# gssales/gaussian-splatting-reflection

Measured on AMD Instinct MI355X. Metric: train_step_views_per_s (fwd+bwd, 1e6 Gaussians @1080p, surfel rasterizer + reflection path), higher is better.
Workload: dtype f32

## Files before the change

gaussian-splatting-reflection_amd/csrc/gsr_common.hip:

```cpp
#include "gsr_internal.hpp"
#include <cstdarg>
#include <string>
#include <initializer_list>
#include <vector>
#include <mutex>
#include "gsr_sort.hpp"
#include <rocprim/device/device_scan.hpp>
#include <rocprim/iterator/counting_iterator.hpp>
#include <rocprim/iterator/transform_iterator.hpp>

namespace gsr {

static thread_local char g_err[512] = "";
void set_error(const char* fmt, ...) {
	va_list ap;
	va_start(ap, fmt);
	vsnprintf(g_err, sizeof(g_err), fmt, ap);
	va_end(ap);
}


struct ProfRec {
	int stage;
	hipEvent_t e0, e1;
};
static bool g_prof_on = false;
static std::vector<ProfRec*> g_prof_recs;
static std::vector<ProfRec*> g_prof_free;
static std::mutex g_prof_mu;

StageTimer::StageTimer(int stage_, hipStream_t stream_) : stage(stage_), stream(stream_), rec(nullptr) {
	if (!g_prof_on) return;
	std::lock_guard<std::mutex> lk(g_prof_mu);
	ProfRec* r = nullptr;
	if (!g_prof_free.empty()) {
		r = g_prof_free.back();
		g_prof_free.pop_back();
	} else {
		r = new ProfRec();
		if (hipEventCreate(&r->e0) != hipSuccess || hipEventCreate(&r->e1) != hipSuccess) { delete r; return; }
	}
	r->stage = stage;
	(void)hipEventRecord(r->e0, stream);
	rec = r;
}
StageTimer::~StageTimer() {
	if (!rec) return;
	ProfRec* r = (ProfRec*)rec;
	(void)hipEventRecord(r->e1, stream);
	std::lock_guard<std::mutex> lk(g_prof_mu);
	g_prof_recs.push_back(r);
}

static int g_opt_cull = 1;
int option_cull() { return g_opt_cull; }
static int g_opt_dev = 0;
int option_dev() { return g_opt_dev; }
static int g_opt_emit_items = 0;
static int g_opt_mailbox = 1;
static int option_mailbox() { return g_opt_mailbox; }
static int g_opt_sort_driver = GSR_ONESWEEP_DRIVER;
int option_sort_driver() { return GSR_ONESWEEP_DRIVER && g_opt_sort_driver; }

uint32_t higher_msb(uint32_t n) {
	uint32_t msb = sizeof(n) * 4;
	uint32_t step = msb;
	while (step > 1) {
		step /= 2;
		if (n >> msb) msb += step;
		else msb -= step;
	}
	if (n >> msb) msb++;
	return msb;
}

using SortConfig = rocprim::radix_sort_config<rocprim::default_config, rocprim::default_config, rocprim::default_config, 65536>;
#ifndef DEPTH_SORT_BS
#define DEPTH_SORT_BS 1024
#endif
#ifndef DEPTH_SORT_IPT
#define DEPTH_SORT_IPT 4
#endif
#define DEPTH_SORT_SHAPE DEPTH_SORT_BS, DEPTH_SORT_IPT, 8
#define DEPTH_KEY_BITS 31u
#define DEPTH_KEY_PLACES 4u
#ifndef TILE_SORT_IPT
#define TILE_SORT_IPT 16
#endif
#ifndef TILE_SORT_BITS
#define TILE_SORT_BITS 8
#endif
#ifndef TILE_SORT_BS
#define TILE_SORT_BS 1024
#endif
#define TILE_SORT_SHAPE TILE_SORT_BS, TILE_SORT_IPT, TILE_SORT_BITS
#ifndef TILE_SORT_SMALL_FROM
#define TILE_SORT_SMALL_FROM 9000000
#endif
#define TILE_SORT_SHAPE_SMALL TILE_SORT_BS, (TILE_SORT_IPT / 2), TILE_SORT_BITS
#define TILE_SORT_SHAPE_SMALL7 TILE_SORT_BS, (TILE_SORT_IPT / 2), 7
static bool tile_sort_small(size_t R) { return R >= (size_t)TILE_SORT_SMALL_FROM; }
static bool tile_sort_7bit(size_t R, int end_bit) { return tile_sort_small(R) && end_bit > 7 && end_bit <= 14; }
template <class F>
static auto with_tile_sort(size_t R, int end_bit, F&& f) {
	if (tile_sort_7bit(R, end_bit)) return f(RadixSort<TILE_SORT_SHAPE_SMALL7, SortConfig>{});
	if (tile_sort_small(R)) return f(RadixSort<TILE_SORT_SHAPE_SMALL, SortConfig>{});
	return f(RadixSort<TILE_SORT_SHAPE, SortConfig>{});
}
using DepthSort = RadixSort<DEPTH_SORT_SHAPE, SortConfig>;

struct OrderRect {
	const uint32_t* rect;
	int packed;
	__host__ __device__ unsigned long long operator()(uint32_t i) const {
		uint32_t hi = 0u;
// ... 465 lines not shown
int run_tile_order(const ImageState& img, size_t tiles, hipStream_t stream) {
	if (tiles == 0) return 0;
	tile_order_kernel<<<1, 1024, 0, stream>>>((int)tiles, img.ranges, img.tile_order);
	GSR_LAUNCH_CHECK(0, stream);
	return 0;
}

__global__ void __launch_bounds__(256) mark_visible_kernel(int P, const float* __restrict__ pts, const float* __restrict__ vm,
                                                           uint8_t* __restrict__ present) {
#pragma clang fp contract(off)
	const int idx = blockIdx.x * 256 + threadIdx.x;
	if (idx >= P) return;
	const float x = pts[3 * idx], y = pts[3 * idx + 1], z = pts[3 * idx + 2];
	const float pz = vm[2] * x + vm[6] * y + vm[10] * z + vm[14];
	present[idx] = (pz <= 0.2f) ? 0 : 1;
}

__global__ void __launch_bounds__(256) widen_clamped_kernel(int P, const uint8_t* __restrict__ packed, uint8_t* __restrict__ out) {
	const int idx = blockIdx.x * 256 + threadIdx.x;
	if (idx >= P) return;
	const uint8_t b = packed[idx];
	out[3 * idx + 0] = b & 1;
	out[3 * idx + 1] = (b >> 1) & 1;
	out[3 * idx + 2] = (b >> 2) & 1;
}
struct RecPick { int n; int pos[9]; };
__global__ void __launch_bounds__(256) pick_rec_kernel(int P, const float* __restrict__ rec, int stride, RecPick pick, float* __restrict__ out) {
	const int i = blockIdx.x * 256 + threadIdx.x;
	if (i >= P * pick.n) return;
	const int idx = i / pick.n, k = i % pick.n;
	out[i] = rec[(size_t)idx * stride + pick.pos[k]];
}
__global__ void __launch_bounds__(256) gather_rec_kernel(int P, const float* __restrict__ rec, int stride, int first, int nf,
                                                         float* __restrict__ out) {
	const int i = blockIdx.x * 256 + threadIdx.x;
	if (i >= P * nf) return;
	const int idx = i / nf, k = i % nf;
	out[i] = rec[(size_t)idx * stride + first + k];
}

}

using namespace gsr;

extern "C" const char* gsr_last_error(void) { return g_err; }
extern "C" int gsr_version(void) { return GSR_ABI_VERSION; }


extern "C" int gsr_set_option(const char* name, int value) {
	if (std::string(name) == "cull") { g_opt_cull = value ? 1 : 0; return 0; }
	if (std::string(name) == "dev") { g_opt_dev = value; return 0; }
	if (std::string(name) == "emit_items") { g_opt_emit_items = (value == 1 || value == 2) ? value : 0; return 0; }
	if (std::string(name) == "mailbox") { g_opt_mailbox = value ? 1 : 0; return 0; }
	if (std::string(name) == "sort_driver") { g_opt_sort_driver = value ? 1 : 0; return 0; }
	set_error("gsr_set_option: unknown option '%s'", name);
	return GSR_E_INVALID;
}
extern "C" int gsr_profile_enable(int on) {
	std::lock_guard<std::mutex> lk(g_prof_mu);
	for (ProfRec* r : g_prof_recs) g_prof_free.push_back(r);
	g_prof_recs.clear();
	g_prof_on = on != 0;
	return 0;
}
extern "C" int gsr_profile_collect(float* ms_out, int* launches_out) {
	std::lock_guard<std::mutex> lk(g_prof_mu);
	for (int i = 0; i < GSR_STAGE_COUNT; i++) { if (ms_out) ms_out[i] = 0.f; if (launches_out) launches_out[i] = 0; }
	for (ProfRec* r : g_prof_recs) {
		float ms = 0.f;
		if (hipEventSynchronize(r->e1) == hipSuccess && hipEventElapsedTime(&ms, r->e0, r->e1) == hipSuccess) {
			if (ms_out) ms_out[r->stage] += ms;
			if (launches_out) launches_out[r->stage] += 1;
		}
		g_prof_free.push_back(r);
	}
	g_prof_recs.clear();
	return 0;
}

extern "C" int gsr_mark_visible(int P, const float* means3D, const float* viewmatrix, const float* projmatrix, uint8_t* present,
                                void* stream_) {
	(void)projmatrix;
	hipStream_t stream = (hipStream_t)stream_;
	if (P < 0 || (P > 0 && (!means3D || !viewmatrix || !present))) { set_error("gsr_mark_visible: invalid argument"); return GSR_E_INVALID; }
	if (P == 0) return 0;
	mark_visible_kernel<<<(P + 255) / 256, 256, 0, stream>>>(P, means3D, viewmatrix, present);
	GSR_LAUNCH_CHECK(0, stream);
	return 0;
}

extern "C" int gsr_debug_fetch(int variant, const char* name, int P, int R, int width, int height, const void* geom_buffer,
                               const void* binning_buffer, const void* image_buffer, void* dst, void* stream_) {
	hipStream_t stream = (hipStream_t)stream_;
	const int tiles_x = (width + 15) / 16, tiles_y = (height + 15) / 16;
	const size_t HW = (size_t)width * height, tiles = (size_t)tiles_x * tiles_y;
	const WorkspaceLayout& layout = variant == 0 ? SURFEL_LAYOUT : GAUSS_LAYOUT;
	const int stride = layout.rec_f4 * 4;
	GeomState g = carve_geom((void*)geom_buffer, P, layout, nullptr);
	ImageState im = carve_image((void*)image_buffer, HW, tiles, layout, nullptr);
	BinningState b = carve_binning((void*)binning_buffer, R, tiles, 0, nullptr);
	auto d2d = [&](const void* src, size_t bytes) -> int {
		if (bytes == 0) return 0;
		GSR_HIP_CHECK(hipMemcpyAsync(dst, src, bytes, hipMemcpyDeviceToDevice, stream));
		return 0;
	};
	auto gather = [&](int first, int nf) -> int {
// ... 53 lines not shown
```

gaussian-splatting-reflection_amd/csrc/gsr_internal.hpp:

```cpp
#pragma once
#include <cstring>
#include <cstdint>
#include <cstdio>
#include <hip/hip_runtime.h>
#include "../../include/gsr_hip.h"

#define GSR_TILE 16
#define GSR_TILE_PIX 256

namespace gsr {

void set_error(const char* fmt, ...);
#define GSR_HIP_CHECK(expr)                                                                       \
	do {                                                                                          \
		hipError_t _e = (expr);                                                                   \
		if (_e != hipSuccess) {                                                                   \
			gsr::set_error("%s failed: %s (%s:%d)", #expr, hipGetErrorString(_e), __FILE__, __LINE__); \
			return GSR_E_HIP;                                                                     \
		}                                                                                         \
	} while (0)
#define GSR_LAUNCH_CHECK(debug, stream)                                  \
	do {                                                                 \
		GSR_HIP_CHECK(hipGetLastError());                                \
		if (debug) GSR_HIP_CHECK(hipStreamSynchronize(stream));          \
// ... 79 lines not shown
constexpr WorkspaceLayout SURFEL_LAYOUT{S_REC_F4, 0, S_ACC_F, 3, 2};
constexpr WorkspaceLayout GAUSS_LAYOUT{G_REC_F4, 0, G_ACC_F, 1, 1};

GeomState carve_geom(void* buf, size_t P, const WorkspaceLayout& layout, size_t* total);
ImageState carve_image(void* buf, size_t HW, size_t tiles, const WorkspaceLayout& layout, size_t* total);
BinningState carve_binning(void* buf, size_t R, size_t tiles, size_t sort_temp_bytes, size_t* total, bool blend_masks = true);
int forward_workspace(gsr_alloc_fn alloc, void* alloc_user, const WorkspaceLayout& layout, size_t P, size_t HW, size_t tiles, GeomState* geom,
                      ImageState* img);

static inline int check_sh_input(const char* entry, int D, int M, const float* shs) {
	if (D < 0 || D > 3 || (shs && (D + 1) * (D + 1) > M)) { set_error("%s: SH degree %d not supported with M=%d", entry, D, M); return GSR_E_INVALID; }
	if (shs && ((M * 3) & 3) == 0 && misaligned16(shs)) {
		set_error("%s: shs (rows of a multiple of 16 bytes) must be 16-byte aligned (float4 accesses); got %p", entry, (const void*)shs);
		return GSR_E_INVALID;
	}
	return 0;
}

struct RasterCam {
	const float* view;
	const float* proj;
	const float* campos;
	int W, H;
	float tan_fovx, tan_fovy, focal_x, focal_y;
};
static inline RasterCam make_cam(const float* view, const float* proj, const float* campos, int W, int H, float tan_fovx, float tan_fovy) {
	RasterCam c;
	c.view = view; c.proj = proj; c.campos = campos; c.W = W; c.H = H;
	c.tan_fovx = tan_fovx; c.tan_fovy = tan_fovy;
	c.focal_y = H / (2.0f * tan_fovy);
	c.focal_x = W / (2.0f * tan_fovx);
	return c;
}

struct BackwardWorkspace { GeomState geom; ImageState img; BinningState bin; int tiles_x, ntiles; };
static inline int backward_prologue(const char* entry, const char* func, const WorkspaceLayout& layout, int P, int M, int R, int width, int height,
                                    bool missing_pointer, const float* shs, const float* dL_dsh, const float* dL_drot, const float* also_aligned,
                                    const char* also_what, void* geom_buffer, void* binning_buffer, void* image_buffer, hipStream_t stream,
                                    BackwardWorkspace* w) {
	if (P < 0 || R < 0 || width <= 0 || height <= 0) { set_error("%s: invalid size", entry); return GSR_E_INVALID; }
	if (P == 0) return 0;
	if (missing_pointer) { set_error("%s: missing required pointer", entry); return GSR_E_INVALID; }
	if (shs && ((M * 3) & 3) == 0) GSR_REQUIRE_ALIGNED16_IN(func, shs, "shs (rows of a multiple of 16 bytes)");
	if (shs && ((M * 3) & 3) == 0) GSR_REQUIRE_ALIGNED16_IN(func, dL_dsh, "dL_dsh");
	GSR_REQUIRE_ALIGNED16_IN(func, dL_drot, "dL_drot");
	GSR_REQUIRE_ALIGNED16_IN(func, also_aligned, also_what);
	w->tiles_x = (width + 15) / 16;
	w->ntiles = w->tiles_x * ((height + 15) / 16);
	w->geom = carve_geom(geom_buffer, P, layout, nullptr);
	w->img = carve_image(image_buffer, (size_t)width * height, w->ntiles, layout, nullptr);
	w->bin = carve_binning(binning_buffer, R, w->ntiles, 0, nullptr);
	GSR_HIP_CHECK(hipMemsetAsync(w->geom.acc, 0, (size_t)P * layout.acc_floats * sizeof(float), stream));
	return 1;
}

int option_cull();
int option_dev();
size_t sort_temp_bytes(size_t R, int end_bit);
int run_tile_order(const ImageState& img, size_t tiles, hipStream_t stream);
uint32_t higher_msb(uint32_t n);

int run_binning(gsr_alloc_fn alloc, void* alloc_user, int P, int tiles_x, int tiles_y, const GeomState& geom,
                const ImageState& img, BinningState* out_binning, int prefiltered, int debug, hipStream_t stream, bool blend_masks = true);

int side_gate_wait(hipStream_t stream);
int refl_sort_keys_early(uint32_t L, int width, int height, float* scratch, size_t scratch_floats, const uint32_t* sort_keys, int async, bool gated,
                         hipStream_t stream);

}

#ifdef __HIPCC__
namespace gsr {

__device__ __forceinline__ int f2i(float v) { return (int)v; }

__device__ __forceinline__ void get_rect(float px, float py, int max_radius, int gx, int gy, uint32_t& x0, uint32_t& y0,
                                         uint32_t& x1, uint32_t& y1) {
	const float r = (float)max_radius;
	x0 = (uint32_t)min(gx, max(0, f2i((px - r) / 16.0f)));
	y0 = (uint32_t)min(gy, max(0, f2i((py - r) / 16.0f)));
	x1 = (uint32_t)min(gx, max(0, f2i((px + r + 15.0f) / 16.0f)));
	y1 = (uint32_t)min(gy, max(0, f2i((py + r + 15.0f) / 16.0f)));
}

#define GSR_DPP1(CTRL, i) "v_add_f32_dpp %" #i ", %" #i ", %" #i " " CTRL "\n\t"
#define GSR_DPP4(CTRL) GSR_DPP1(CTRL, 0) GSR_DPP1(CTRL, 1) GSR_DPP1(CTRL, 2) GSR_DPP1(CTRL, 3)
#define GSR_SHR1 "row_shr:1 row_mask:0xf bank_mask:0xf bound_ctrl:0"
#define GSR_SHR2 "row_shr:2 row_mask:0xf bank_mask:0xf bound_ctrl:0"
#define GSR_SHR4 "row_shr:4 row_mask:0xf bank_mask:0xf bound_ctrl:0"
#define GSR_SHR8 "row_shr:8 row_mask:0xf bank_mask:0xf bound_ctrl:0"
#define GSR_BC15 "row_bcast:15 row_mask:0xa bank_mask:0xf"
#define GSR_BC31 "row_bcast:31 row_mask:0xc bank_mask:0xf"
__device__ __forceinline__ void wave_sum4(float* v) {
	asm volatile("s_nop 1\n\t" GSR_DPP4(GSR_SHR1) GSR_DPP4(GSR_SHR2) GSR_DPP4(GSR_SHR4) GSR_DPP4(GSR_SHR8) GSR_DPP4(GSR_BC15) GSR_DPP4(GSR_BC31)
	             : "+v"(v[0]), "+v"(v[1]), "+v"(v[2]), "+v"(v[3]));
}

#define GSR_Q1(CTRL, i) "v_add_f32_dpp %" #i ", %" #i ", %" #i " " CTRL " row_mask:0xf bank_mask:0xf\n\t"
#define GSR_DPPB(CTRL, BANK, dst, src) "v_add_f32_dpp %" #dst ", %" #src ", %" #src " " CTRL " row_mask:0xf bank_mask:" BANK "\n\t"
#define GSR_L1(CTRL, d, a, b) GSR_DPPB(CTRL, "0x3", d, a) GSR_DPPB(CTRL, "0xc", d, b)
__device__ __forceinline__ void row_reduce20(const float* v, float* z) {
	float p0, q0, p1, q1, p2, q2, p3, q3, p4, q4;
	asm volatile("s_nop 1\n\t" GSR_L1("row_mirror", 0, 6, 7) GSR_L1("row_mirror", 1, 8, 9) GSR_L1("row_mirror", 2, 10, 11)
	             GSR_L1("row_mirror", 3, 12, 13) GSR_L1("row_mirror", 4, 14, 15) GSR_L1("row_mirror", 5, 16, 17)
	             : "=&v"(p0), "=&v"(q0), "=&v"(p1), "=&v"(q1), "=&v"(p2), "=&v"(q2)
	             : "v"(v[0]), "v"(v[1]), "v"(v[2]), "v"(v[3]), "v"(v[4]), "v"(v[5]), "v"(v[6]), "v"(v[7]), "v"(v[8]), "v"(v[9]), "v"(v[10]), "v"(v[11]));
// ... 202 lines not shown
```

gaussian-splatting-reflection_amd/csrc/gsr_surfel.hip:

```cpp
#include <type_traits>
#include "gsr_internal.hpp"
#include "gsr_tile_walk.hpp"
#include "gsr_sort.hpp"
#include "gsr_math.hpp"
#include "gsr_refl.hpp"

namespace gsr {

#define SA_COLOR 0
#define SA_REFL 3
#define SA_NORMAL 4
#define SA_OPAC 7
#define SA_T 8
#define SA_MEAN2D 17

#define S_NEAR 0.2f
#define S_FAR 100.0f
#define S_FILTER_INV_SQ 2.0f

__device__ __forceinline__ M3 quat_to_rotmat(const float* __restrict__ q, float& w, float& x, float& y, float& z) {
#pragma clang fp contract(off)
	const float s = 1.0f / sqrtf(q[3] * q[3] + q[0] * q[0] + q[1] * q[1] + q[2] * q[2]);
	w = q[0] * s; x = q[1] * s; y = q[2] * s; z = q[3] * s;
	return m3_make(1.f - 2.f * (y * y + z * z), 2.f * (x * y + w * z), 2.f * (x * z - w * y), 2.f * (x * y - w * z),
// ... 24 lines not shown
	float qw, qx, qy, qz;
	const M3 R = quat_to_rotmat(rot, qw, qx, qy, qz);
	const float s0 = mod * scale[0], s1 = mod * scale[1];
	const float L0[3] = {R.m[0][0] * s0, R.m[0][1] * s0, R.m[0][2] * s0};
	const float L1[3] = {R.m[1][0] * s1, R.m[1][1] * s1, R.m[1][2] * s1};
	const float* pm = cam.proj;
	float AB[4][3];
#pragma unroll
	for (int j = 0; j < 4; j++) {
		AB[j][0] = L0[0] * pm[j] + L0[1] * pm[j + 4] + L0[2] * pm[j + 8];
		AB[j][1] = L1[0] * pm[j] + L1[1] * pm[j + 4] + L1[2] * pm[j + 8];
		AB[j][2] = px * pm[j] + py * pm[j + 4] + pz * pm[j + 8] + pm[j + 12];
	}
	const float Wh = (float)(float(cam.W) / 2.0), Wm = (float)(float(cam.W - 1) / 2.0);
	const float Hh = (float)(float(cam.H) / 2.0), Hm = (float)(float(cam.H - 1) / 2.0);
#pragma unroll
	for (int i = 0; i < 3; i++) {
		T.m[0][i] = AB[0][i] * Wh + AB[3][i] * Wm;
		T.m[1][i] = AB[1][i] * Hh + AB[3][i] * Hm;
		T.m[2][i] = AB[3][i];
	}
	const float* vm = cam.view;
	const float nx = R.m[2][0], ny = R.m[2][1], nz = R.m[2][2];
	normal = f3(vm[0] * nx + vm[4] * ny + vm[8] * nz, vm[1] * nx + vm[5] * ny + vm[9] * nz, vm[2] * nx + vm[6] * ny + vm[10] * nz);
}

__device__ __forceinline__ void surfel_cull_record(const M3& T, float cx, float cy, float opa, float4& c0, float4& c1) {
	c0 = make_float4(cx, cy, 0.f, 0.f);
	c1 = make_float4(0.f, cx, cy, -2.0f);
	if (!(opa >= 1.0f / 255.0f)) return;
	const float c2f = 2.0f * logf(255.0f * opa) * 1.05f + 0.1f;
	c1.w = 0.5f * c2f * 1.02f;
	const double ic2 = 1.0 / (double)c2f;
	const double a00 = T.m[0][0], a01 = T.m[0][1], a02 = T.m[0][2];
	const double a10 = T.m[1][0], a11 = T.m[1][1], a12 = T.m[1][2];
	const double a20 = T.m[2][0], a21 = T.m[2][1], a22 = T.m[2][2];
	const double sigma = a20 * a20 + a21 * a21 - a22 * a22 * ic2;
	if (!(sigma < -1e-6 * a22 * a22 * ic2)) return;
	const double sx = a00 * a20 + a01 * a21 - a02 * a22 * ic2, sy = a10 * a20 + a11 * a21 - a12 * a22 * ic2;
	const double Sxx = a00 * a00 + a01 * a01 - a02 * a02 * ic2, Sxy = a00 * a10 + a01 * a11 - a02 * a12 * ic2,
	             Syy = a10 * a10 + a11 * a11 - a12 * a12 * ic2;
	const double is = 1.0 / sigma;
	const double ex = sx * is, ey = sy * is;
	const double g = -is * 1.0404;
	const double Vxx = (Sxx - sx * sx * is) * g + 0.25, Vxy = (Sxy - sx * sy * is) * g, Vyy = (Syy - sy * sy * is) * g + 0.25;
	const double det = Vxx * Vyy - Vxy * Vxy;
	if (!(Vxx > 0.25) || !(Vyy > 0.25) || !(det > 0.0)) return;
	const float fa = (float)(Vyy / det), fb = (float)(-Vxy / det), fc = (float)(Vxx / det);
	if (!(fa > 0.f) || !(fc > 0.f) || !(fa * fc - fb * fb > 0.f) || !(fabsf((float)ex) < 1e7f) || !(fabsf((float)ey) < 1e7f)) return;
	c0 = make_float4((float)ex, (float)ey, fa, fb);
	c1.x = fc;
}

template <bool TRAIN>
__device__ __forceinline__ bool
surfel_preprocess_one(int idx, int D, int M, const float* __restrict__ means, const float* __restrict__ scales, float scale_modifier,
                      const float* __restrict__ rotations, const float* __restrict__ opacities, const float* __restrict__ shs,
                      const float* __restrict__ transMat_precomp, const float* __restrict__ colors_precomp, const float* __restrict__ refl,
                      const uint8_t* __restrict__ env_scope_mask, const RasterCam& cam, int* __restrict__ radii, const GeomState& g, int gx, int gy,
                      int prefiltered, float* __restrict__ gaussian_weights, float4* o) {
#pragma clang fp contract(off)
	radii[idx] = 0;
	if constexpr (TRAIN) gaussian_weights[idx] = 0.f;
	g.tiles_touched[idx] = 0;
	reinterpret_cast<uint2*>(g.rect)[idx] = make_uint2(0u, 0u);
	g.depths[idx] = __int_as_float(0x7f7fffff);
	const float mx = means[3 * idx], my = means[3 * idx + 1], mz = means[3 * idx + 2];
	const float* vm = cam.view;
	const float pvx = vm[0] * mx + vm[4] * my + vm[8] * mz + vm[12];
	const float pvy = vm[1] * mx + vm[5] * my + vm[9] * mz + vm[13];
	const float pvz = vm[2] * mx + vm[6] * my + vm[10] * mz + vm[14];
	if (pvz <= 0.2f) {
		if (prefiltered) g.flags[0] = 1;
		return false;
	}
	M3 T;
	F3 normal;
	if (transMat_precomp == nullptr) {
		compute_transmat(mx, my, mz, scales + 2 * idx, scale_modifier, rotations + 4 * idx, cam, T, normal);
	} else {
#pragma unroll
		for (int c = 0; c < 3; c++)
#pragma unroll
			for (int r = 0; r < 3; r++) T.m[c][r] = transMat_precomp[9 * idx + 3 * c + r];
		normal = f3(0.0f, 0.0f, 1.0f);
	}
	const float cosv = -((pvx * normal.x) + (pvy * normal.y) + (pvz * normal.z));
	if (cosv == 0) return false;
	const float multiplier = cosv > 0 ? 1.f : -1.f;
	normal = f3(multiplier * normal.x, multiplier * normal.y, multiplier * normal.z);
	const float cutoff = 3.0f;
	const float t0 = cutoff * cutoff, t1 = cutoff * cutoff, t2 = -1.0f;
	const float d = t0 * (T.m[2][0] * T.m[2][0]) + t1 * (T.m[2][1] * T.m[2][1]) + t2 * (T.m[2][2] * T.m[2][2]);
	if (d == 0.0f) return false;
	const float inv_d = 1 / d;
	const float f0 = inv_d * t0, f1 = inv_d * t1, f2 = inv_d * t2;
	const float pxi = f0 * (T.m[0][0] * T.m[2][0]) + f1 * (T.m[0][1] * T.m[2][1]) + f2 * (T.m[0][2] * T.m[2][2]);
	const float pyi = f0 * (T.m[1][0] * T.m[2][0]) + f1 * (T.m[1][1] * T.m[2][1]) + f2 * (T.m[1][2] * T.m[2][2]);
	const float h0x = pxi * pxi - (f0 * (T.m[0][0] * T.m[0][0]) + f1 * (T.m[0][1] * T.m[0][1]) + f2 * (T.m[0][2] * T.m[0][2]));
	const float h0y = pyi * pyi - (f0 * (T.m[1][0] * T.m[1][0]) + f1 * (T.m[1][1] * T.m[1][1]) + f2 * (T.m[1][2] * T.m[1][2]));
	const float ex = sqrtf(fmaxf(1e-4f, h0x)), ey = sqrtf(fmaxf(1e-4f, h0y));
	const float radius = ceilf(fmaxf(fmaxf(ex, ey), cutoff * (float)0.707106));
	uint32_t x0, y0, x1, y1;
	get_rect(pxi, pyi, f2i(radius), gx, gy, x0, y0, x1, y1);
	if ((x1 - x0) * (y1 - y0) == 0) return false;

	float cr, cg, cb;
	if (colors_precomp == nullptr) {
		const float dx = mx - cam.campos[0], dy = my - cam.campos[1], dz = mz - cam.campos[2];
		const float len = sqrtf(dx * dx + dy * dy + dz * dz);
		ShRow s;
		load_sh(shs, idx, M, (D + 1) * (D + 1), s);
		const F3 c = sh_eval(D, s, dx / len, dy / len, dz / len);
		if constexpr (TRAIN) g.clamped[idx] = (uint8_t)((c.x < 0 ? 1 : 0) | (c.y < 0 ? 2 : 0) | (c.z < 0 ? 4 : 0));
		cr = fmaxf(c.x, 0.0f); cg = fmaxf(c.y, 0.0f); cb = fmaxf(c.z, 0.0f);
	} else {
		cr = colors_precomp[3 * idx]; cg = colors_precomp[3 * idx + 1]; cb = colors_precomp[3 * idx + 2];
	}
	g.depths[idx] = pvz;
	radii[idx] = f2i(radius);
	g.rect[2 * idx] = x0 | (y0 << 16);
	g.rect[2 * idx + 1] = x1 | (y1 << 16);
	const float maskv = (env_scope_mask != nullptr && env_scope_mask[idx]) ? 1.0f : 0.0f;
	surfel_cull_record(T, pxi, pyi, opacities[idx], o[5], o[6]);
	float4* rec = o;
	rec[0] = make_float4(pxi, pyi, T.m[0][0], T.m[1][0]);
	rec[1] = make_float4(T.m[0][1], T.m[1][1], T.m[0][2], T.m[1][2]);
	rec[2] = make_float4(T.m[2][0], T.m[2][1], T.m[2][2], opacities[idx]);
	rec[3] = make_float4(normal.x, normal.y, normal.z, refl[idx]);
	rec[4] = make_float4(cr, cg, cb, maskv);
	g.tiles_touched[idx] = (y1 - y0) * (x1 - x0);
	return true;
}

#define S_OUT_F4 7
struct CubemapInterleave {
	const float* cubemap;
	float4* rgba;
	uint32_t ntex, LL;
};
template <bool TRAIN>
__global__ void __launch_bounds__(256)
surfel_preprocess_kernel(int P, int D, int M, const float* __restrict__ means, const float* __restrict__ scales, float scale_modifier,
                         const float* __restrict__ rotations, const float* __restrict__ opacities, const float* __restrict__ shs,
                         const float* __restrict__ transMat_precomp, const float* __restrict__ colors_precomp,
                         const float* __restrict__ refl, const uint8_t* __restrict__ env_scope_mask, RasterCam cam, int* __restrict__ radii,
                         GeomState g, int gx, int gy, int prefiltered, float* __restrict__ gaussian_weights, CubemapInterleave ci) {
	const int idx = blockIdx.x * 256 + threadIdx.x;
	for (uint32_t t = (uint32_t)idx; t < ci.ntex; t += gridDim.x * 256u) {
		const uint32_t f = t / ci.LL, r = t - f * ci.LL;
		const float* c = ci.cubemap + (size_t)f * 3 * ci.LL + r;
		ci.rgba[t] = make_float4(c[0], c[ci.LL], c[2 * (size_t)ci.LL], 0.f);
	}
	sort_clear_region(g.depth_sort_temp, g.depth_sort_clear, (size_t)idx, (size_t)gridDim.x * 256u);
	sort_clear_region(g.emit_state, g.emit_state_bytes, (size_t)idx, (size_t)gridDim.x * 256u);
	if (idx == 0) { g.flags[1] = 0; g.flags[2] = 0; g.flags[3] = 0; }
	__shared__ float4 s_out[4][S_REC_F4 * 65];
	const int lane = threadIdx.x & 63;
	float4* so = s_out[threadIdx.x >> 6];
	float4 o[S_OUT_F4];
#pragma unroll
	for (int k = 0; k < S_OUT_F4; k++) o[k] = make_float4(0.f, 0.f, 0.f, 0.f);
	bool live = false;
	if (idx < P)
		live = surfel_preprocess_one<TRAIN>(idx, D, M, means, scales, scale_modifier, rotations, opacities, shs, transMat_precomp, colors_precomp, refl,
		                             env_scope_mask, cam, radii, g, gx, gy, prefiltered, gaussian_weights, o);
	if (__ballot(live) == 0ull) return;
	const int g0 = idx - lane;
	const int ng = min(64, P - g0);
	wave_store_rows4<S_REC_F4, false>(so, o, g.rec + (size_t)g0 * S_REC_F4, S_REC_F4, 0, ng, lane);
	wave_store_rows4<2, false>(so, o + S_REC_F4, g.bbox + (size_t)g0 * 2, 2, 0, ng, lane);
}

typedef float v2f __attribute__((ext_vector_type(2)));
__device__ __forceinline__ v2f mk2(float a, float b) { v2f r; r.x = a; r.y = b; return r; }

struct SurfelRec : TileRec<S_REC_F4> {
	__device__ __forceinline__ v2f xy() const { return mk2(f[0].x, f[0].y); }
	__device__ __forceinline__ v2f TuvX() const { return mk2(f[0].z, f[0].w); }
	__device__ __forceinline__ v2f TuvY() const { return mk2(f[1].x, f[1].y); }
	__device__ __forceinline__ v2f TuvZ() const { return mk2(f[1].z, f[1].w); }
	__device__ __forceinline__ v2f Twxy() const { return mk2(f[2].x, f[2].y); }
	__device__ __forceinline__ float Twz() const { return f[2].z; }
	__device__ __forceinline__ float opac() const { return f[2].w; }
	__device__ __forceinline__ v2f nxy() const { return mk2(f[3].x, f[3].y); }
	__device__ __forceinline__ float nz() const { return f[3].z; }
	__device__ __forceinline__ float refl() const { return f[3].w; }
	__device__ __forceinline__ v2f rg() const { return mk2(f[4].x, f[4].y); }
	__device__ __forceinline__ float b() const { return f[4].z; }
	__device__ __forceinline__ float mask() const { return f[4].w; }
};

#ifndef GSR_BWD_WPE
#define GSR_BWD_WPE 4
#endif
#ifndef GSR_BWD_LIST
#define GSR_BWD_LIST 1
#endif
#ifndef GSR_BWD_UNROLL
#define GSR_BWD_UNROLL 1
#endif
#ifdef GSR_FWD_WPE
#define GSR_FWD_ATTR __attribute__((amdgpu_waves_per_eu(GSR_FWD_WPE, GSR_FWD_WPE)))
#else
#define GSR_FWD_ATTR
#endif

struct SurfelFwdPix {
	float T, C2, M2, distortion, median_depth, median_contributor, maskacc;
	v2f Crg, Nxy, NzR, DM;
	uint32_t last_contributor;
};

template <bool TRAIN>
__device__ __forceinline__ lmask surfel_fwd_pair(const SurfelRec& R, const v2f pix, uint32_t contributor, bool med_live, SurfelFwdPix& st,
                                                 lmask& done, float& wq, bool& grazed) {
	float sx, sy, rho3d, depth, alpha, rho2d;
	{
#pragma clang fp contract(off)
		const v2f Tw = R.Twxy();
		const v2f X = pix * Tw.x - R.TuvX();
		const v2f Y = pix * Tw.y - R.TuvY();
		const v2f Z = pix * R.Twz() - R.TuvZ();
		const v2f a = Y * Z.yx;
// ... 748 lines not shown
		return GSR_E_INVALID;
	}
	return check_sh_input(entry, D, M, shs);
}

static int early_key_sort(const gsr_refl_forward* refl, int width, int height, int R, hipStream_t stream) {
	if (!refl || !refl->sort_keys || !refl->scratch) return 0;
	return refl_sort_keys_early(refl->L, width, height, refl->scratch, refl->scratch_floats, refl->sort_keys, refl->async_sort, R > 0, stream);
}

template <bool TRAIN>
static int surfel_forward(gsr_alloc_fn alloc, void* alloc_user, int P, int D, int M, const float* background, int width, int height,
                          const float* means3D, const uint8_t* env_scope_mask, const float* shs, const float* colors_precomp,
                          const float* refl_strengths, const float* opacities, const float* scales, float scale_modifier,
                          const float* rotations, const float* transMat_precomp, const float* viewmatrix, const float* projmatrix,
                          const float* cam_pos, float tan_fovx, float tan_fovy, int prefiltered, float* out_color, float* out_others,
                          float* out_alpha, float* out_normal_view, float* out_refl_strength_map, int* radii, float* gaussian_weights,
                          const gsr_refl_forward* refl, int debug, hipStream_t stream) {
	const size_t HW = (size_t)width * height;
	int R = 0;
	if (P == 0) {
		float* normal = TRAIN ? out_others + 2 * HW : out_normal_view;
		if (!normal) {
			normal = static_cast<float*>(alloc(alloc_user, GSR_BUF_IMAGE, HW * 3 * 4));
			if (!normal) { set_error("workspace allocation failed (%zu bytes)", HW * 3 * 4); return GSR_E_ALLOC; }
		}
		GSR_HIP_CHECK(hipMemsetAsync(out_color, 0, HW * 3 * 4, stream));
		if (TRAIN) {
			GSR_HIP_CHECK(hipMemsetAsync(out_others, 0, HW * 8 * 4, stream));
		} else {
			GSR_HIP_CHECK(hipMemsetAsync(out_alpha, 0, HW * 4, stream));
			GSR_HIP_CHECK(hipMemsetAsync(normal, 0, HW * 3 * 4, stream));
		}
		GSR_HIP_CHECK(hipMemsetAsync(out_refl_strength_map, 0, HW * 4, stream));
		if (refl && gsr_deferred_reflection_forward_keys(normal, out_color, out_refl_strength_map, refl->cam, refl->cubemap, refl->fail_value, refl->L,
		                                                 width, height, refl->out_final, refl->out_refl_color, refl->out_normal_world, refl->cubemap_rgba,
		                                                 refl->sort_keys, stream) < 0)
			return GSR_E_HIP;
	} else {
		const int tiles_x = (width + 15) / 16, tiles_y = (height + 15) / 16;
		const int ntiles = tiles_x * tiles_y;
		GeomState geom; ImageState img;
		if (const int rc = forward_workspace(alloc, alloc_user, TRAIN ? SURFEL_LAYOUT : SURFEL_LAYOUT.inference(), P, HW, ntiles, &geom, &img); rc < 0) return rc;

		if (prefiltered) GSR_HIP_CHECK(hipMemsetAsync(geom.flags, 0, 4 * sizeof(int), stream));
		const RasterCam cam = make_cam(viewmatrix, projmatrix, cam_pos, width, height, tan_fovx, tan_fovy);
		CubemapInterleave ci{nullptr, nullptr, 0u, 1u};
		SurfelReflFwd rf{};
		if (refl) {
			ci = CubemapInterleave{refl->cubemap, reinterpret_cast<float4*>(refl->cubemap_rgba), 6u * refl->L * refl->L, refl->L * refl->L};
			rf = SurfelReflFwd{refl->cam, refl->cubemap, reinterpret_cast<const float4*>(refl->cubemap_rgba), refl->fail_value, (int)refl->L, 6u * refl->L * refl->L,
			                   refl->out_final, refl->out_refl_color, refl->out_normal_world, refl->sort_keys};
		}
	{ StageTimer st_(GSR_STAGE_PREPROCESS, stream); 	surfel_preprocess_kernel<TRAIN><<<(P + 255) / 256, 256, 0, stream>>>(P, D, M, means3D, scales, scale_modifier, rotations, opacities, shs,
		                                                                     transMat_precomp, colors_precomp, refl_strengths, env_scope_mask, cam, radii, geom,
		                                                                     tiles_x, tiles_y, prefiltered, gaussian_weights, ci); }
		GSR_LAUNCH_CHECK(debug, stream);

		BinningState bin;
		R = run_binning(alloc, alloc_user, P, tiles_x, tiles_y, geom, img, &bin, prefiltered, debug, stream, TRAIN);
		if (R < 0) return R;

	{ StageTimer st_(GSR_STAGE_RENDER_FWD, stream);
		const int nunits = (int)xcd_grid((uint32_t)ntiles * 4u);
		const auto args = [&] { if constexpr (TRAIN) return rf; else return SurfelEvalFwd{rf, out_alpha, out_normal_view}; }();
		auto render = refl ? surfel_render_fwd_wave_kernel<true, TRAIN> : surfel_render_fwd_wave_kernel<false, TRAIN>;
		render<<<nunits, 64, 0, stream>>>(img.ranges, img.tile_order, bin.point_list, width, height, tiles_x, ntiles, geom.rec, geom.bbox, option_cull(),
		                                  background, TRAIN ? img.final_T : nullptr, TRAIN ? img.n_contrib : nullptr, out_color, out_others,
		                                  out_refl_strength_map, gaussian_weights, bin.blend_mask, bin.mask_stride, args); }
		GSR_LAUNCH_CHECK(debug, stream);
	}
	if (const int rc = TRAIN ? early_key_sort(refl, width, height, R, stream) : 0; rc < 0) return rc;
	return R;
}

extern "C" int gsr_surfel_forward_refl(gsr_alloc_fn alloc, void* alloc_user, int P, int D, int M, const float* background, int width, int height,
                                  const float* means3D, const uint8_t* env_scope_mask, const float* shs, const float* colors_precomp,
                                  const float* refl_strengths, const float* opacities, const float* scales, float scale_modifier,
                                  const float* rotations, const float* transMat_precomp, const float* viewmatrix, const float* projmatrix,
                                  const float* cam_pos, float tan_fovx, float tan_fovy, int prefiltered, float* out_color, float* out_others,
                                  float* out_refl_strength_map, int* radii, float* gaussian_weights, const gsr_refl_forward* refl, int debug,
                                  void* stream_) {
	if (!alloc || P < 0 || width <= 0 || height <= 0 || !background || !out_color || !out_others || !out_refl_strength_map) {
		set_error("gsr_surfel_forward: invalid argument");
		return GSR_E_INVALID;
	}
	if (P > 0 && !gaussian_weights) { set_error("gsr_surfel_forward: missing required input pointer"); return GSR_E_INVALID; }
	if (const int rc = check_refl_descriptor("gsr_surfel_forward_refl", refl); rc < 0) return rc;
	if (const int rc = check_surfel_inputs("gsr_surfel_forward", P, D, M, means3D, shs, colors_precomp, refl_strengths, opacities, scales, rotations,
	                                       transMat_precomp, viewmatrix, projmatrix, cam_pos, radii); rc < 0) return rc;
	return surfel_forward<true>(alloc, alloc_user, P, D, M, background, width, height, means3D, env_scope_mask, shs, colors_precomp, refl_strengths,
	                            opacities, scales, scale_modifier, rotations, transMat_precomp, viewmatrix, projmatrix, cam_pos, tan_fovx, tan_fovy,
	                            prefiltered, out_color, out_others, nullptr, nullptr, out_refl_strength_map, radii, gaussian_weights, refl, debug,
	                            (hipStream_t)stream_);
}

extern "C" int gsr_surfel_forward(gsr_alloc_fn alloc, void* alloc_user, int P, int D, int M, const float* background, int width, int height,
                                  const float* means3D, const uint8_t* env_scope_mask, const float* shs, const float* colors_precomp,
                                  const float* refl_strengths, const float* opacities, const float* scales, float scale_modifier,
                                  const float* rotations, const float* transMat_precomp, const float* viewmatrix, const float* projmatrix,
                                  const float* cam_pos, float tan_fovx, float tan_fovy, int prefiltered, float* out_color, float* out_others,
                                  float* out_refl_strength_map, int* radii, float* gaussian_weights, int debug, void* stream_) {
	return gsr_surfel_forward_refl(alloc, alloc_user, P, D, M, background, width, height, means3D, env_scope_mask, shs, colors_precomp, refl_strengths, opacities,
	                               scales, scale_modifier, rotations, transMat_precomp, viewmatrix, projmatrix, cam_pos, tan_fovx, tan_fovy, prefiltered, out_color,
	                               out_others, out_refl_strength_map, radii, gaussian_weights, nullptr, debug, stream_);
}

extern "C" int gsr_surfel_forward_eval(gsr_alloc_fn alloc, void* alloc_user, int P, int D, int M, const float* background, int width, int height,
                                       const float* means3D, const float* shs, const float* colors_precomp, const float* refl_strengths,
                                       const float* opacities, const float* scales, float scale_modifier, const float* rotations,
                                       const float* transMat_precomp, const float* viewmatrix, const float* projmatrix, const float* cam_pos,
                                       float tan_fovx, float tan_fovy, int prefiltered, float* out_color, float* out_alpha,
                                       float* out_normal_view, float* out_refl_strength_map, int* radii, const gsr_refl_forward* refl,
                                       int debug, void* stream_) {
// ... 81 lines not shown
```

Measured before the change: 547.2.

## Split surfel preprocess into geometry and shading kernels overlapped on side stream

Preprocessing is split into a light geometry kernel (depths, radii, rects, tiles touched) that binning needs and a shading kernel (SH eval, record packing, cubemap interleave). The shading kernel runs on a pooled low-priority side stream with a capped grid-stride grid, overlapping with binning, and is joined before the forward render. This hides shading latency behind the sort and scan, at the cost of recomputing the transform matrix in both kernels and extra event and stream overhead.

```diff
diff --git a/gaussian-splatting-reflection_amd/csrc/gsr_common.hip b/gaussian-splatting-reflection_amd/csrc/gsr_common.hip
--- a/gaussian-splatting-reflection_amd/csrc/gsr_common.hip
+++ b/gaussian-splatting-reflection_amd/csrc/gsr_common.hip
@@ -4,6 +4,8 @@
 #include <initializer_list>
 #include <vector>
 #include <mutex>
+#include <algorithm>
+#include <utility>
 #include "gsr_sort.hpp"
 #include <rocprim/device/device_scan.hpp>
 #include <rocprim/iterator/counting_iterator.hpp>
@@ -61,6 +63,69 @@
 static int option_mailbox() { return g_opt_mailbox; }
 static int g_opt_sort_driver = GSR_ONESWEEP_DRIVER;
 int option_sort_driver() { return GSR_ONESWEEP_DRIVER && g_opt_sort_driver; }
+
+static int g_opt_shade_async = 1;
+int option_shade_async() { return g_opt_shade_async; }
+static int g_opt_shade_grid = 0;
+unsigned shade_grid_size(int P, int cap) {
+	const int blocks = (P + 255) / 256, want = g_opt_shade_grid > 0 ? g_opt_shade_grid : cap;
+	return (unsigned)std::max(1, std::min(blocks, want));
+}
+
+#ifndef FWD_SIDE_PRIO_HIGH
+#define FWD_SIDE_PRIO_HIGH 0
+#endif
+namespace {
+struct ForwardSideSet {
+	hipStream_t stream;
+	hipEvent_t fork, done;
+};
+std::mutex g_fwd_side_mu;
+std::vector<ForwardSideSet> g_fwd_side[64];
+}
+
+int ForwardSide::fork(bool async) {
+	if (!async || side) return 0;
+	if (hipGetDevice(&dev) != hipSuccess || dev < 0 || dev >= 64) { set_error("forward side stream: no current device"); return GSR_E_HIP; }
+	std::lock_guard<std::mutex> lk(g_fwd_side_mu);
+	std::vector<ForwardSideSet>& pool = g_fwd_side[dev];
+	if (pool.empty()) {
+		ForwardSideSet n{nullptr, nullptr, nullptr};
+		int least = 0, greatest = 0;
+		GSR_HIP_CHECK(hipDeviceGetStreamPriorityRange(&least, &greatest));
+		GSR_HIP_CHECK(hipStreamCreateWithPriority(&n.stream, hipStreamNonBlocking, FWD_SIDE_PRIO_HIGH ? greatest : least));
+		if (hipEventCreateWithFlags(&n.fork, hipEventDisableTiming) != hipSuccess || hipEventCreateWithFlags(&n.done, hipEventDisableTiming) != hipSuccess) {
+			if (n.fork) (void)hipEventDestroy(n.fork);
+			(void)hipStreamDestroy(n.stream);
+			set_error("forward side stream: event creation failed");
+			return GSR_E_HIP;
+		}
+		pool.push_back(n);
+	}
+	side = pool.back().stream; ev_fork = pool.back().fork; ev_done = pool.back().done;
+	pool.pop_back();
+	GSR_HIP_CHECK(hipEventRecord(ev_fork, caller));
+	GSR_HIP_CHECK(hipStreamWaitEvent(side, ev_fork, 0));
+	return 0;
+}
+int ForwardSide::launched() {
+	if (!side || done_recorded) return 0;
+	GSR_HIP_CHECK(hipEventRecord(ev_done, side));
+	done_recorded = true;
+	return 0;
+}
+int ForwardSide::join() {
+	if (!side) return 0;
+	hipError_t e = done_recorded ? hipSuccess : hipEventRecord(ev_done, side);
+	if (e == hipSuccess) e = hipStreamWaitEvent(caller, ev_done, 0);
+	{
+		std::lock_guard<std::mutex> lk(g_fwd_side_mu);
+		g_fwd_side[dev].push_back(ForwardSideSet{side, ev_fork, ev_done});
+	}
+	side = nullptr;
+	if (e != hipSuccess) { set_error("forward side stream: join failed: %s", hipGetErrorString(e)); return GSR_E_HIP; }
+	return 0;
+}
 
 uint32_t higher_msb(uint32_t n) {
 	uint32_t msb = sizeof(n) * 4;
@@ -632,6 +697,8 @@
 	if (std::string(name) == "dev") { g_opt_dev = value; return 0; }
 	if (std::string(name) == "emit_items") { g_opt_emit_items = (value == 1 || value == 2) ? value : 0; return 0; }
 	if (std::string(name) == "mailbox") { g_opt_mailbox = value ? 1 : 0; return 0; }
+	if (std::string(name) == "shade_async") { g_opt_shade_async = value ? 1 : 0; return 0; }
+	if (std::string(name) == "shade_grid") { g_opt_shade_grid = value > 0 ? value : 0; return 0; }
 	if (std::string(name) == "sort_driver") { g_opt_sort_driver = value ? 1 : 0; return 0; }
 	set_error("gsr_set_option: unknown option '%s'", name);
 	return GSR_E_INVALID;
diff --git a/gaussian-splatting-reflection_amd/csrc/gsr_internal.hpp b/gaussian-splatting-reflection_amd/csrc/gsr_internal.hpp
--- a/gaussian-splatting-reflection_amd/csrc/gsr_internal.hpp
+++ b/gaussian-splatting-reflection_amd/csrc/gsr_internal.hpp
@@ -155,6 +155,43 @@
 	w->bin = carve_binning(binning_buffer, R, w->ntiles, 0, nullptr);
 	GSR_HIP_CHECK(hipMemsetAsync(w->geom.acc, 0, (size_t)P * layout.acc_floats * sizeof(float), stream));
 	return 1;
+}
+
+class ForwardSide {
+	hipStream_t caller, side = nullptr;
+	hipEvent_t ev_fork = nullptr, ev_done = nullptr;
+	int dev = 0;
+	bool done_recorded = false;
+public:
+	explicit ForwardSide(hipStream_t caller_) : caller(caller_) {}
+	ForwardSide(const ForwardSide&) = delete;
+	ForwardSide& operator=(const ForwardSide&) = delete;
+	~ForwardSide() { (void)join(); }
+	int fork(bool async);
+	hipStream_t lane() const { return side ? side : caller; }
+	int launched();
+	int join();
+};
+int option_shade_async();
+unsigned shade_grid_size(int P, int cap);
+
+#ifndef SHADE_GRID
+#define SHADE_GRID 256
+#endif
+template <class Geometry, class Shade>
+static inline int run_split_preprocess(ForwardSide& side, int debug, hipStream_t stream, Geometry&& geometry, Shade&& shade) {
+	{
+		StageTimer st_(GSR_STAGE_SCAN, stream);
+		geometry(stream);
+	}
+	GSR_LAUNCH_CHECK(debug, stream);
+	if (const int rc = side.fork(option_shade_async() && !debug); rc < 0) return rc;
+	{
+		StageTimer st_(GSR_STAGE_PREPROCESS, side.lane());
+		shade(side.lane());
+	}
+	GSR_LAUNCH_CHECK(debug, stream);
+	return side.launched();
 }
 
 int option_cull();
diff --git a/gaussian-splatting-reflection_amd/csrc/gsr_surfel.hip b/gaussian-splatting-reflection_amd/csrc/gsr_surfel.hip
--- a/gaussian-splatting-reflection_amd/csrc/gsr_surfel.hip
+++ b/gaussian-splatting-reflection_amd/csrc/gsr_surfel.hip
@@ -100,29 +100,32 @@
 	c1.x = fc;
 }
 
-template <bool TRAIN>
+struct SurfelGeomOut {
+	float mx, my, mz;
+	float pvz;
+	float pxi, pyi;
+	M3 T;
+	F3 normal;
+	float radius;
+	uint32_t x0, y0, x1, y1;
+};
 __device__ __forceinline__ bool
-surfel_preprocess_one(int idx, int D, int M, const float* __restrict__ means, const float* __restrict__ scales, float scale_modifier,
-                      const float* __restrict__ rotations, const float* __restrict__ opacities, const float* __restrict__ shs,
-                      const float* __restrict__ transMat_precomp, const float* __restrict__ colors_precomp, const float* __restrict__ refl,
-                      const uint8_t* __restrict__ env_scope_mask, const RasterCam& cam, int* __restrict__ radii, const GeomState& g, int gx, int gy,
-                      int prefiltered, float* __restrict__ gaussian_weights, float4* o) {
+surfel_geometry_one(int idx, const float* __restrict__ means, const float* __restrict__ scales, float scale_modifier, const float* __restrict__ rotations,
+                    const float* __restrict__ transMat_precomp, const RasterCam& cam, int gx, int gy, bool& behind, SurfelGeomOut& s) {
 #pragma clang fp contract(off)
-	radii[idx] = 0;
-	if constexpr (TRAIN) gaussian_weights[idx] = 0.f;
-	g.tiles_touched[idx] = 0;
-	reinterpret_cast<uint2*>(g.rect)[idx] = make_uint2(0u, 0u);
-	g.depths[idx] = __int_as_float(0x7f7fffff);
+	behind = false;
 	const float mx = means[3 * idx], my = means[3 * idx + 1], mz = means[3 * idx + 2];
+	s.mx = mx; s.my = my; s.mz = mz;
 	const float* vm = cam.view;
 	const float pvx = vm[0] * mx + vm[4] * my + vm[8] * mz + vm[12];
 	const float pvy = vm[1] * mx + vm[5] * my + vm[9] * mz + vm[13];
 	const float pvz = vm[2] * mx + vm[6] * my + vm[10] * mz + vm[14];
 	if (pvz <= 0.2f) {
-		if (prefiltered) g.flags[0] = 1;
+		behind = true;
 		return false;
 	}
-	M3 T;
+	s.pvz = pvz;
+	M3& T = s.T;
 	F3 normal;
 	if (transMat_precomp == nullptr) {
 		compute_transmat(mx, my, mz, scales + 2 * idx, scale_modifier, rotations + 4 * idx, cam, T, normal);
@@ -136,7 +139,7 @@
 	const float cosv = -((pvx * normal.x) + (pvy * normal.y) + (pvz * normal.z));
 	if (cosv == 0) return false;
 	const float multiplier = cosv > 0 ? 1.f : -1.f;
-	normal = f3(multiplier * normal.x, multiplier * normal.y, multiplier * normal.z);
+	s.normal = f3(multiplier * normal.x, multiplier * normal.y, multiplier * normal.z);
 	const float cutoff = 3.0f;
 	const float t0 = cutoff * cutoff, t1 = cutoff * cutoff, t2 = -1.0f;
 	const float d = t0 * (T.m[2][0] * T.m[2][0]) + t1 * (T.m[2][1] * T.m[2][1]) + t2 * (T.m[2][2] * T.m[2][2]);
@@ -148,36 +151,65 @@
 	const float h0x = pxi * pxi - (f0 * (T.m[0][0] * T.m[0][0]) + f1 * (T.m[0][1] * T.m[0][1]) + f2 * (T.m[0][2] * T.m[0][2]));
 	const float h0y = pyi * pyi - (f0 * (T.m[1][0] * T.m[1][0]) + f1 * (T.m[1][1] * T.m[1][1]) + f2 * (T.m[1][2] * T.m[1][2]));
 	const float ex = sqrtf(fmaxf(1e-4f, h0x)), ey = sqrtf(fmaxf(1e-4f, h0y));
-	const float radius = ceilf(fmaxf(fmaxf(ex, ey), cutoff * (float)0.707106));
-	uint32_t x0, y0, x1, y1;
-	get_rect(pxi, pyi, f2i(radius), gx, gy, x0, y0, x1, y1);
-	if ((x1 - x0) * (y1 - y0) == 0) return false;
-
+	s.radius = ceilf(fmaxf(fmaxf(ex, ey), cutoff * (float)0.707106));
+	s.pxi = pxi; s.pyi = pyi;
+	get_rect(pxi, pyi, f2i(s.radius), gx, gy, s.x0, s.y0, s.x1, s.y1);
+	return (s.x1 - s.x0) * (s.y1 - s.y0) != 0;
+}
+
+template <bool TRAIN>
+__global__ void __launch_bounds__(256)
+surfel_geometry_kernel(int P, const float* __restrict__ means, const float* __restrict__ scales, float scale_modifier, const float* __restrict__ rotations,
+                       const float* __restrict__ transMat_precomp, RasterCam cam, int* __restrict__ radii, GeomState g, int gx, int gy, int prefiltered,
+                       float* __restrict__ gaussian_weights) {
+	const int idx = blockIdx.x * 256 + threadIdx.x;
+	sort_clear_region(g.depth_sort_temp, g.depth_sort_clear, (size_t)idx, (size_t)gridDim.x * 256u);
+	sort_clear_region(g.emit_state, g.emit_state_bytes, (size_t)idx, (size_t)gridDim.x * 256u);
+	if (idx == 0) { g.flags[1] = 0; g.flags[2] = 0; g.flags[3] = 0; }
+	if (idx >= P) return;
+	SurfelGeomOut s;
+	bool behind;
+	const bool live = surfel_geometry_one(idx, means, scales, scale_modifier, rotations, transMat_precomp, cam, gx, gy, behind, s);
+	if (behind && prefiltered) g.flags[0] = 1;
+	if constexpr (TRAIN) gaussian_weights[idx] = 0.f;
+	radii[idx] = live ? f2i(s.radius) : 0;
+	g.tiles_touched[idx] = live ? (s.y1 - s.y0) * (s.x1 - s.x0) : 0u;
+	reinterpret_cast<uint2*>(g.rect)[idx] = live ? make_uint2(s.x0 | (s.y0 << 16), s.x1 | (s.y1 << 16)) : make_uint2(0u, 0u);
+	g.depths[idx] = live ? s.pvz : __int_as_float(0x7f7fffff);
+}
+
+template <bool TRAIN>
+__device__ __forceinline__ bool
+surfel_shade_one(int idx, int D, int M, const float* __restrict__ means, const float* __restrict__ scales, float scale_modifier,
+                 const float* __restrict__ rotations, const float* __restrict__ opacities, const float* __restrict__ shs,
+                 const float* __restrict__ transMat_precomp, const float* __restrict__ colors_precomp, const float* __restrict__ refl,
+                 const uint8_t* __restrict__ env_scope_mask, const RasterCam& cam, const GeomState& g, int gx, int gy, float4* o) {
+#pragma clang fp contract(off)
+	SurfelGeomOut s;
+	bool behind;
+	if (!surfel_geometry_one(idx, means, scales, scale_modifier, rotations, transMat_precomp, cam, gx, gy, behind, s)) return false;
+	const M3& T = s.T;
 	float cr, cg, cb;
 	if (colors_precomp == nullptr) {
-		const float dx = mx - cam.campos[0], dy = my - cam.campos[1], dz = mz - cam.campos[2];
+		const float dx = s.mx - cam.campos[0], dy = s.my - cam.campos[1], dz = s.mz - cam.campos[2];
 		const float len = sqrtf(dx * dx + dy * dy + dz * dz);
-		ShRow s;
-		load_sh(shs, idx, M, (D + 1) * (D + 1), s);
-		const F3 c = sh_eval(D, s, dx / len, dy / len, dz / len);
+		ShRow sh;
+		load_sh(shs, idx, M, (D + 1) * (D + 1), sh);
+		const F3 c = sh_eval(D, sh, dx / len, dy / len, dz / len);
 		if constexpr (TRAIN) g.clamped[idx] = (uint8_t)((c.x < 0 ? 1 : 0) | (c.y < 0 ? 2 : 0) | (c.z < 0 ? 4 : 0));
 		cr = fmaxf(c.x, 0.0f); cg = fmaxf(c.y, 0.0f); cb = fmaxf(c.z, 0.0f);
 	} else {
 		cr = colors_precomp[3 * idx]; cg = colors_precomp[3 * idx + 1]; cb = colors_precomp[3 * idx + 2];
 	}
-	g.depths[idx] = pvz;
-	radii[idx] = f2i(radius);
-	g.rect[2 * idx] = x0 | (y0 << 16);
-	g.rect[2 * idx + 1] = x1 | (y1 << 16);
 	const float maskv = (env_scope_mask != nullptr && env_scope_mask[idx]) ? 1.0f : 0.0f;
-	surfel_cull_record(T, pxi, pyi, opacities[idx], o[5], o[6]);
+	const float opa = opacities[idx];
+	surfel_cull_record(T, s.pxi, s.pyi, opa, o[5], o[6]);
 	float4* rec = o;
-	rec[0] = make_float4(pxi, pyi, T.m[0][0], T.m[1][0]);
+	rec[0] = make_float4(s.pxi, s.pyi, T.m[0][0], T.m[1][0]);
 	rec[1] = make_float4(T.m[0][1], T.m[1][1], T.m[0][2], T.m[1][2]);
-	rec[2] = make_float4(T.m[2][0], T.m[2][1], T.m[2][2], opacities[idx]);
-	rec[3] = make_float4(normal.x, normal.y, normal.z, refl[idx]);
+	rec[2] = make_float4(T.m[2][0], T.m[2][1], T.m[2][2], opa);
+	rec[3] = make_float4(s.normal.x, s.normal.y, s.normal.z, refl[idx]);
 	rec[4] = make_float4(cr, cg, cb, maskv);
-	g.tiles_touched[idx] = (y1 - y0) * (x1 - x0);
 	return true;
 }
 
@@ -189,35 +221,33 @@
 };
 template <bool TRAIN>
 __global__ void __launch_bounds__(256)
-surfel_preprocess_kernel(int P, int D, int M, const float* __restrict__ means, const float* __restrict__ scales, float scale_modifier,
-                         const float* __restrict__ rotations, const float* __restrict__ opacities, const float* __restrict__ shs,
-                         const float* __restrict__ transMat_precomp, const float* __restrict__ colors_precomp,
-                         const float* __restrict__ refl, const uint8_t* __restrict__ env_scope_mask, RasterCam cam, int* __restrict__ radii,
-                         GeomState g, int gx, int gy, int prefiltered, float* __restrict__ gaussian_weights, CubemapInterleave ci) {
-	const int idx = blockIdx.x * 256 + threadIdx.x;
-	for (uint32_t t = (uint32_t)idx; t < ci.ntex; t += gridDim.x * 256u) {
+surfel_shade_kernel(int P, int D, int M, const float* __restrict__ means, const float* __restrict__ scales, float scale_modifier,
+                    const float* __restrict__ rotations, const float* __restrict__ opacities, const float* __restrict__ shs,
+                    const float* __restrict__ transMat_precomp, const float* __restrict__ colors_precomp, const float* __restrict__ refl,
+                    const uint8_t* __restrict__ env_scope_mask, RasterCam cam, GeomState g, int gx, int gy, CubemapInterleave ci) {
+	for (uint32_t t = blockIdx.x * 256u + threadIdx.x; t < ci.ntex; t += gridDim.x * 256u) {
 		const uint32_t f = t / ci.LL, r = t - f * ci.LL;
 		const float* c = ci.cubemap + (size_t)f * 3 * ci.LL + r;
 		ci.rgba[t] = make_float4(c[0], c[ci.LL], c[2 * (size_t)ci.LL], 0.f);
 	}
-	sort_clear_region(g.depth_sort_temp, g.depth_sort_clear, (size_t)idx, (size_t)gridDim.x * 256u);
-	sort_clear_region(g.emit_state, g.emit_state_bytes, (size_t)idx, (size_t)gridDim.x * 256u);
-	if (idx == 0) { g.flags[1] = 0; g.flags[2] = 0; g.flags[3] = 0; }
 	__shared__ float4 s_out[4][S_REC_F4 * 65];
 	const int lane = threadIdx.x & 63;
 	float4* so = s_out[threadIdx.x >> 6];
-	float4 o[S_OUT_F4];
-#pragma unroll
-	for (int k = 0; k < S_OUT_F4; k++) o[k] = make_float4(0.f, 0.f, 0.f, 0.f);
-	bool live = false;
-	if (idx < P)
-		live = surfel_preprocess_one<TRAIN>(idx, D, M, means, scales, scale_modifier, rotations, opacities, shs, transMat_precomp, colors_precomp, refl,
-		                             env_scope_mask, cam, radii, g, gx, gy, prefiltered, gaussian_weights, o);
-	if (__ballot(live) == 0ull) return;
-	const int g0 = idx - lane;
-	const int ng = min(64, P - g0);
-	wave_store_rows4<S_REC_F4, false>(so, o, g.rec + (size_t)g0 * S_REC_F4, S_REC_F4, 0, ng, lane);
-	wave_store_rows4<2, false>(so, o + S_REC_F4, g.bbox + (size_t)g0 * 2, 2, 0, ng, lane);
+	for (long long base = (long long)blockIdx.x * 256; base < (long long)P; base += (long long)gridDim.x * 256) {
+		const int idx = (int)base + (int)threadIdx.x;
+		float4 o[S_OUT_F4];
+#pragma unroll
+		for (int k = 0; k < S_OUT_F4; k++) o[k] = make_float4(0.f, 0.f, 0.f, 0.f);
+		bool live = false;
+		if (idx < P)
+			live = surfel_shade_one<TRAIN>(idx, D, M, means, scales, scale_modifier, rotations, opacities, shs, transMat_precomp, colors_precomp, refl,
+			                               env_scope_mask, cam, g, gx, gy, o);
+		if (__ballot(live) == 0ull) continue;
+		const int g0 = idx - lane;
+		const int ng = min(64, P - g0);
+		wave_store_rows4<S_REC_F4, false>(so, o, g.rec + (size_t)g0 * S_REC_F4, S_REC_F4, 0, ng, lane);
+		wave_store_rows4<2, false>(so, o + S_REC_F4, g.bbox + (size_t)g0 * 2, 2, 0, ng, lane);
+	}
 }
 
 typedef float v2f __attribute__((ext_vector_type(2)));
@@ -1072,14 +1102,22 @@
 			rf = SurfelReflFwd{refl->cam, refl->cubemap, reinterpret_cast<const float4*>(refl->cubemap_rgba), refl->fail_value, (int)refl->L, 6u * refl->L * refl->L,
 			                   refl->out_final, refl->out_refl_color, refl->out_normal_world, refl->sort_keys};
 		}
-	{ StageTimer st_(GSR_STAGE_PREPROCESS, stream); 	surfel_preprocess_kernel<TRAIN><<<(P + 255) / 256, 256, 0, stream>>>(P, D, M, means3D, scales, scale_modifier, rotations, opacities, shs,
-		                                                                     transMat_precomp, colors_precomp, refl_strengths, env_scope_mask, cam, radii, geom,
-		                                                                     tiles_x, tiles_y, prefiltered, gaussian_weights, ci); }
-		GSR_LAUNCH_CHECK(debug, stream);
+		ForwardSide side(stream);
+		if (const int rc = run_split_preprocess(side, debug, stream,
+		        [&](hipStream_t s) {
+			        surfel_geometry_kernel<TRAIN><<<(P + 255) / 256, 256, 0, s>>>(P, means3D, scales, scale_modifier, rotations, transMat_precomp, cam, radii, geom,
+			                                                                      tiles_x, tiles_y, prefiltered, gaussian_weights);
+		        },
+		        [&](hipStream_t s) {
+			        surfel_shade_kernel<TRAIN><<<shade_grid_size(P, SHADE_GRID), 256, 0, s>>>(P, D, M, means3D, scales, scale_modifier, rotations, opacities, shs,
+			                                                                            transMat_precomp, colors_precomp, refl_strengths, env_scope_mask, cam, geom,
+			                                                                            tiles_x, tiles_y, ci);
+		        }); rc < 0) return rc;
 
 		BinningState bin;
 		R = run_binning(alloc, alloc_user, P, tiles_x, tiles_y, geom, img, &bin, prefiltered, debug, stream, TRAIN);
 		if (R < 0) return R;
+		if (const int rc = side.join(); rc < 0) return rc;
 
 	{ StageTimer st_(GSR_STAGE_RENDER_FWD, stream);
 		const int nunits = (int)xcd_grid((uint32_t)ntiles * 4u);
```

New measurement: 554.5 (median of 6 runs). +1.3%, better.
